# alevar/tiebrush

Hardware: AMD Instinct MI355X
Metric: input alignment records/sec collapsed (tiebrush) + bases/sec covered (tiecov) (higher is better)
Workload: dtype int64; 1 GPU; c3: 64 synthetic sorted BAMs x 5000000 100bp reads per GPU, --clip collapse + tiecov -c -j of the result; records_per_gpu=320000000, groups_out=25086541, parallelism=files-per-rank x1, ranks_seen=1, resident=SoA in HBM before the timed region, contexts=3

## Files before the change

### tiebrush_amd/csrc/collapse.hip

```cpp
#include <stdlib.h>

#include <chrono>

#include "dev_common.hpp"
#include "rx_w64.hpp"
#include "scan_op.hpp"
#include "strategy.hpp"
#include "tbk_internal.h"
#include "wgroup.h"

namespace {

struct EffKey {
  uint32_t khi_h, khi_l;
  int32_t kend;
  uint32_t flag_cnt;
};
struct EffOp {
  __device__ __forceinline__ EffKey operator()(const EffKey& a, const EffKey& b) const {
    uint64_t ak = ((uint64_t)a.khi_h << 32) | a.khi_l, bk = ((uint64_t)b.khi_h << 32) | b.khi_l;
    bool take_b = (b.flag_cnt >> 31) || bk > ak || (bk == ak && b.kend > a.kend);
    EffKey r;
    r.khi_h = take_b ? b.khi_h : a.khi_h;
    r.khi_l = take_b ? b.khi_l : a.khi_l;
// ... 354 lines not shown
  if (i >= n) return;
  const uint32_t sg = rec_sg[i];
  rec_group[i] = sg == 0xFFFFFFFFu ? -1 : (int32_t)ginv[sg];
}


constexpr uint32_t YS_NT = 1024;
constexpr uint32_t YS_NL = 128;
struct YsIn {
  uint32_t ng;
  const uint32_t* gperm;
  const uint32_t* ns;
  const uint32_t* gpoff;
  const uint16_t* pfile;
  const uint64_t* ghi;
  const uint64_t* gfmask;
};
__device__ __forceinline__ uint64_t ys_spread32(uint64_t x) {
  x = (x | (x << 16)) & 0x0000FFFF0000FFFFull;
  x = (x | (x << 8)) & 0x00FF00FF00FF00FFull;
  x = (x | (x << 4)) & 0x0F0F0F0F0F0F0F0Full;
  x = (x | (x << 2)) & 0x3333333333333333ull;
  x = (x | (x << 1)) & 0x5555555555555555ull;
  return x;
}
__device__ __forceinline__ void ys_mask_from_files(uint64_t files, uint32_t c, uint64_t* lo, uint64_t* hi) {
  const uint64_t a = ys_spread32(files & 0xFFFFFFFFull), b = ys_spread32(files >> 32);
  *lo = c == 0u ? a : (c == 1u ? a << 1 : (a | (a << 1)));
  *hi = c == 0u ? b : (c == 1u ? b << 1 : (b | (b << 1)));
}
__device__ __forceinline__ uint64_t wave_bit_transpose(uint64_t x) {
  const uint32_t lane = lane_id();
#define YS_TSTEP(J, M)                                                                     \
  {                                                                                        \
    const uint64_t tt = ((uint64_t)(uint32_t)__shfl_xor((int)(uint32_t)(x >> 32), J, 64) << 32) | (uint32_t)__shfl_xor((int)(uint32_t)x, J, 64); \
    x = (lane & J) ? (((tt >> J) & M) | (x & ~M)) : ((x & M) | ((tt & M) << J));           \
  }
  YS_TSTEP(32, 0x00000000FFFFFFFFull)
  YS_TSTEP(16, 0x0000FFFF0000FFFFull)
  YS_TSTEP(8, 0x00FF00FF00FF00FFull)
  YS_TSTEP(4, 0x0F0F0F0F0F0F0F0Full)
  YS_TSTEP(2, 0x3333333333333333ull)
  YS_TSTEP(1, 0x5555555555555555ull)
#undef YS_TSTEP
  return x;
}
struct YsAgg {
  uint32_t first_tid, last_tid;
  int32_t mx;
  uint32_t whole;
};
__device__ __forceinline__ YsAgg ys_combine(const YsAgg& a, const YsAgg& b) {
  if (b.last_tid == 0u) return a;
  if (a.last_tid == 0u) return b;
  YsAgg r;
  r.first_tid = a.first_tid;
  r.last_tid = b.last_tid;
  const bool joins = b.whole && b.first_tid == a.last_tid;
  r.mx = joins ? (a.mx > b.mx ? a.mx : b.mx) : b.mx;
  r.whole = joins ? a.whole : 0u;
  return r;
}
struct YsCells {
  uint32_t (*a)[YS_NL];
  uint32_t (*b)[YS_NL];
  int32_t (*m)[YS_NL];
  __device__ __forceinline__ YsAgg get(uint32_t x, uint32_t c) const { return YsAgg{a[x][c] & 0x7FFFFFFFu, b[x][c], m[x][c], a[x][c] >> 31}; }
  __device__ __forceinline__ void put(uint32_t x, uint32_t c, const YsAgg& v) const {
    a[x][c] = v.first_tid | (v.whole << 31);
    b[x][c] = v.last_tid;
    m[x][c] = v.mx;
  }
};
__device__ __forceinline__ YsAgg ys_chain_cells(const YsCells& P, uint32_t c, YsAgg run) {
  for (uint32_t x = 0; x < YS_NT / 64; ++x) {
    const YsAgg mine = P.get(x, c);
    P.put(x, c, run);
    run = ys_combine(run, mine);
  }
  return run;
}
__global__ __launch_bounds__(YS_NT) void yd_lcount_k(YsIn S, const uint4* __restrict__ gpk , uint32_t ntiles,
                                                     uint32_t* __restrict__ table , uint4* __restrict__ agg ,
                                                     uint64_t* __restrict__ gfiles ) {
  __shared__ uint64_t wb[YS_NT / 64][YS_NL];
  __shared__ uint32_t g_tid[YS_NT];
  __shared__ int32_t g_e1[YS_NT];
  __shared__ uint32_t pa[YS_NT / 64][YS_NL], pb[YS_NT / 64][YS_NL];
  __shared__ int32_t pm[YS_NT / 64][YS_NL];
  const YsCells P{pa, pb, pm};
  uint64_t lo = 0, hi = 0;
  {
    const uint32_t o = blockIdx.x * YS_NT + threadIdx.x;
    if (o < S.ng) {
      const uint32_t sg = S.gperm[o];
      const uint32_t c = (uint32_t)S.ghi[sg] & 3u;
      const uint32_t n = S.gfmask ? 0u : S.ns[sg], p0 = S.gfmask ? 0u : S.gpoff[sg];
      uint64_t files = 0;
      if (S.gfmask)
        files = S.gfmask[sg];
      else
        for (uint32_t i = 0; i < n; ++i) files |= 1ull << S.pfile[p0 + i];
      gfiles[2 * (size_t)o] = files;
      gfiles[2 * (size_t)o + 1] = c;
      ys_mask_from_files(files, c, &lo, &hi);
      const uint4 g = gpk[o];
      g_tid[threadIdx.x] = g.x;
      g_e1[threadIdx.x] = (int32_t)g.z + 1;
    }
  }
  wb[threadIdx.x >> 6][lane_id()] = wave_bit_transpose(lo);
  wb[threadIdx.x >> 6][64u + lane_id()] = wave_bit_transpose(hi);
  __syncthreads();
  for (uint32_t q = threadIdx.x; q < (YS_NT / 64) * YS_NL; q += YS_NT) {
    const uint32_t x = q / YS_NL, c = q % YS_NL;
    YsAgg A{0u, 0u, INT32_MIN, 1u};
    for (uint64_t m = wb[x][c]; m; m &= m - 1) {
      const uint32_t g = x * 64u + (uint32_t)__builtin_ctzll(m);
      A = ys_combine(A, YsAgg{g_tid[g], g_tid[g], g_e1[g], 1u});
    }
    P.put(x, c, A);
  }
  __syncthreads();
  if (threadIdx.x < YS_NL) {
    const uint32_t c = threadIdx.x;
    uint32_t n = 0;
    for (uint32_t x = 0; x < YS_NT / 64; ++x) n += (uint32_t)__builtin_popcountll(wb[x][c]);
    const YsAgg A = ys_chain_cells(P, c, YsAgg{0u, 0u, INT32_MIN, 1u});
    table[(size_t)c * ntiles + blockIdx.x] = n;
    agg[(size_t)c * ntiles + blockIdx.x] = make_uint4(A.first_tid, A.last_tid, (uint32_t)A.mx, A.whole);
  }
}
__global__ __launch_bounds__(256) void yd_lagg_scan_k(uint4* __restrict__ agg, uint32_t ntiles) {
  __shared__ uint4 part[256];
  uint4* row = agg + (size_t)blockIdx.x * ntiles;
  const uint32_t per = (ntiles + 255u) / 256u, i0 = threadIdx.x * per, i1 = i0 + per < ntiles ? i0 + per : ntiles;
  auto un = [](const uint4& v) { return YsAgg{v.x, v.y, (int32_t)v.z, v.w}; };
  auto pk = [](const YsAgg& a) { return make_uint4(a.first_tid, a.last_tid, (uint32_t)a.mx, a.whole); };
  YsAgg A{0u, 0u, INT32_MIN, 1u};
  for (uint32_t i = i0; i < i1; ++i) A = ys_combine(A, un(row[i]));
  part[threadIdx.x] = pk(A);
  __syncthreads();
  if (threadIdx.x == 0) {
    YsAgg run{0u, 0u, INT32_MIN, 1u};
    for (uint32_t q = 0; q < 256; ++q) {
      const YsAgg mine = un(part[q]);
      part[q] = pk(run);
      run = ys_combine(run, mine);
    }
  }
  __syncthreads();
  YsAgg run = un(part[threadIdx.x]);
  for (uint32_t i = i0; i < i1; ++i) {
    const YsAgg mine = un(row[i]);
    row[i] = pk(run);
    run = ys_combine(run, mine);
  }
}
__global__ __launch_bounds__(1024) void yd_lscan_k(uint32_t* __restrict__ table, uint32_t ntiles, uint64_t* __restrict__ totals,
                                                   unsigned long long* __restrict__ nit ) {
  __shared__ uint32_t sm[16];
  __shared__ uint32_t carry_s;
  uint32_t* row = table + (size_t)blockIdx.x * ntiles;
  constexpr uint32_t E = 8;
  if (threadIdx.x == 0) carry_s = 0;
  __syncthreads();
  for (uint32_t base = 0; base < ntiles; base += 1024 * E) {
    const uint32_t i0 = base + threadIdx.x * E;
    uint32_t v[E], s = 0;
#pragma unroll
    for (uint32_t e = 0; e < E; ++e) {
      v[e] = i0 + e < ntiles ? row[i0 + e] : 0u;
      s += v[e];
    }
    uint32_t tot;
    uint32_t ex = carry_s + block_excl_sum<uint32_t, 1024>(s, sm, &tot);
#pragma unroll
    for (uint32_t e = 0; e < E; ++e) {
      if (i0 + e < ntiles) row[i0 + e] = ex;
      ex += v[e];
    }
    __syncthreads();
    if (threadIdx.x == 0) carry_s += tot;
    __syncthreads();
  }
  if (threadIdx.x == 0) {
    totals[blockIdx.x] = carry_s;
    atomicAdd(nit, (unsigned long long)carry_s);
  }
}

struct YdWords {
  const uint64_t* w64;
  const uint32_t* w32;
  __device__ __forceinline__ uint32_t group(uint32_t t) const { return w32 ? w32[t] : (uint32_t)w64[t]; }
};
struct YdItems {
  uint4* pk;
  uint32_t* nex;
  uint2* se = nullptr;
  const uint32_t* gxoff = nullptr;
  __device__ __forceinline__ uint4 rec(uint32_t t) const {
    if (se) {
      const uint2 a = se[t];
      return make_uint4(0u, a.x, a.y, 0u);
    }
    return pk[t];
  }
  __device__ __forceinline__ uint32_t xo_of(const uint4& it, uint32_t group) const { return se ? gxoff[group] : it.w; }
  __device__ __forceinline__ uint32_t tidp1(uint32_t t) const { return reinterpret_cast<const uint32_t*>(pk)[4 * (size_t)t]; }
  __device__ __forceinline__ int32_t start(uint32_t t) const { return (int32_t) reinterpret_cast<const uint32_t*>(pk)[4 * (size_t)t + 1]; }
// ... 19 lines not shown
  *s1 = 0;
  if ((h32 >> 30) == 2u) {
    const uint32_t op = h32 & 0xFu;
    return (op == C_M || op == C_D || op == 7u || op == 8u || op == 0xFu) ? 1u : 0u;
  }
  if ((h32 >> 30) == 3u) {
    const uint32_t a = (h32 >> 20) & 0x3FFu, g = h32 & 0xFFFFFu;
    *e0 = st + a - 1u;
    *s1 = st + a + g;
    return 2u;
  }
  return 0u;
}

__global__ void yd_groups_k(ColIn I, uint32_t ng, const uint32_t* __restrict__ gperm, GroupAcc G, const uint64_t* __restrict__ shi,
                            const uint64_t* __restrict__ slo, YdGroups Q) {
  uint32_t o = blockIdx.x * blockDim.x + threadIdx.x;
  if (o >= ng) return;
  uint32_t sg = gperm[o];
  uint32_t q = G.first[sg];
  uint64_t h = shi[q], l = slo[q];
  int32_t st = (int32_t)(uint32_t)((h >> 2) & 0x7FFFFFFFull);
  const uint32_t tidp1 = (uint32_t)(h >> 33);
  const uint32_t en = (uint32_t)(st + (int32_t)(uint32_t)(l >> 32) - 1);
  uint32_t e0, s1;
  const uint32_t nk = yd_exons_from_key(l, (uint32_t)st, en, &e0, &s1);
  int nex = (int)nk;
  if (nex == 0) {
    const uint32_t r = (uint32_t)(G.rep[sg] & 0xFFFFFFFFull);
    walk_exons(I.pos[r], I.cig + I.cig_off[r], I.cig_off[r + 1] - I.cig_off[r], [](int, int) {}, &nex);
  }
  uint32_t xw = (uint32_t)nex;
  if (nk == 2u) {
    const uint32_t a = e0 - (uint32_t)st + 1u, g = s1 - e0 - 1u;
    if (a < (1u << 10) && g < (1u << 20)) xw = YD_X2 | (a << 20) | g;
  }
  Q.nex[o] = yd_nex_far(xw) ? (uint32_t)nex : 0u;
  Q.pk[o] = make_uint4(tidp1, (uint32_t)st, en, xw);
}

__global__ void yd_gexons_k(ColIn I, uint32_t ng, const uint32_t* __restrict__ gperm, GroupAcc G, const uint64_t* __restrict__ slo, YdGroups Q,
                            uint32_t* __restrict__ ex_s, uint32_t* __restrict__ ex_e) {
  uint32_t o = blockIdx.x * blockDim.x + threadIdx.x;
  if (o >= ng) return;
  const uint4 pk = Q.pk[o];
  if (!yd_nex_far(pk.w)) return;
  const uint32_t sg = gperm[o];
  uint32_t w = Q.xoff[o];
  {
    uint32_t e0, s1;
    const uint32_t nk = yd_exons_from_key(slo[G.first[sg]], pk.y, pk.z, &e0, &s1);
    if (nk) {
      ex_s[w] = pk.y;
      ex_e[w] = e0;
      if (nk == 2u) {
        ex_s[w + 1] = s1;
        ex_e[w + 1] = pk.z;
      }
      return;
    }
  }
  uint32_t r = (uint32_t)(G.rep[sg] & 0xFFFFFFFFull);
  int nex = 0;
  walk_exons(I.pos[r], I.cig + I.cig_off[r], I.cig_off[r + 1] - I.cig_off[r],
             [&](int es, int ee) {
               ex_s[w] = (uint32_t)es;
               ex_e[w] = (uint32_t)ee;
               ++w;
             },
             &nex);
}

struct YdEmit {
  YdGroups Q;
  YdItems Y;
  __device__ __forceinline__ void operator()(uint32_t t, uint64_t w) const {
    const uint32_t o = (uint32_t)w;
    const uint4 g = Q.pk[o];
    Y.pk[t] = make_uint4(g.x, g.y, g.z, Q.xoff[o]);
    Y.nex[t] = g.w;
  }
};

__device__ __forceinline__ uint32_t ys_select(uint64_t v, uint32_t r) {
  const uint32_t lo = (uint32_t)v, cl = (uint32_t)__builtin_popcount(lo);
  const bool up = r >= cl;
  const uint32_t w = up ? (uint32_t)(v >> 32) : lo;
  r = up ? r - cl : r;
  uint32_t pos = 0;
#pragma unroll
  for (uint32_t st = 16; st >= 1; st >>= 1) {
    const uint32_t c = (uint32_t)__builtin_popcount((w >> pos) & ((1u << st) - 1u));
    const bool go = r >= c;
    r = go ? r - c : r;
    pos = go ? pos + st : pos;
  }
  return pos + (up ? 32u : 0u);
}
__global__ __launch_bounds__(YS_NT) void yd_lscatter_k(YsIn S, uint32_t ntiles, const uint32_t* __restrict__ table, const uint64_t* __restrict__ totals,
                                                       const uint4* __restrict__ agg, const uint64_t* __restrict__ gfiles, YdGroups Q, YdItems Y,
                                                       uint32_t* __restrict__ item) {
  __shared__ uint32_t base[YS_NL];
  __shared__ uint32_t pre[YS_NL + 1];
  __shared__ uint64_t wb[YS_NT / 64][YS_NL];
  __shared__ uint64_t hb[YS_NT / 64][YS_NL];
  __shared__ uint32_t ltot[YS_NL];
  __shared__ uint32_t lsum[YS_NL];
  __shared__ uint4 grec[YS_NT];
  __shared__ uint32_t gnex[YS_NT];
  __shared__ uint32_t pa[YS_NT / 64][YS_NL], pb[YS_NT / 64][YS_NL];
  __shared__ int32_t pm[YS_NT / 64][YS_NL];
  const YsCells P{pa, pb, pm};
  const uint32_t t = threadIdx.x, w = t >> 6;
  if (t < YS_NL) ltot[t] = (uint32_t)totals[t];
  const uint32_t o = blockIdx.x * YS_NT + t;
  uint64_t lo = 0, hi = 0;
  if (o < S.ng) ys_mask_from_files(gfiles[2 * (size_t)o], (uint32_t)gfiles[2 * (size_t)o + 1], &lo, &hi);
  wb[w][lane_id()] = wave_bit_transpose(lo);
  wb[w][64u + lane_id()] = wave_bit_transpose(hi);
  if (o < S.ng) {
    const uint4 g = Q.pk[o];
    grec[t] = make_uint4(g.x, g.y, g.z, Q.xoff[o]);
    gnex[t] = g.w;
  }
  __syncthreads();
  for (uint32_t q = t; q < (YS_NT / 64) * YS_NL; q += YS_NT) {
    const uint32_t x = q / YS_NL, c = q % YS_NL;
    YsAgg A{0u, 0u, INT32_MIN, 1u};
    for (uint64_t m = wb[x][c]; m; m &= m - 1) {
      const uint4 g = grec[x * 64u + (uint32_t)__builtin_ctzll(m)];
      A = ys_combine(A, YsAgg{g.x, g.x, (int32_t)g.z + 1, 1u});
    }
    P.put(x, c, A);
  }
  __syncthreads();
  if (t < YS_NL) {
    uint32_t b = 0;
    for (uint32_t c = 0; c < t; ++c) b += ltot[c];
    base[t] = b + table[(size_t)t * ntiles + blockIdx.x];
    uint32_t n = 0;
    for (uint32_t x = 0; x < YS_NT / 64; ++x) n += (uint32_t)__builtin_popcountll(wb[x][t]);
    lsum[t] = n;
    const uint4 av = agg[(size_t)t * ntiles + blockIdx.x];
    (void)ys_chain_cells(P, t, YsAgg{av.x, av.y, (int32_t)av.z, av.w});
  }
  __syncthreads();
  for (uint32_t q = t; q < (YS_NT / 64) * YS_NL; q += YS_NT) {
    const uint32_t x = q / YS_NL, c = q % YS_NL;
    YsAgg A = P.get(x, c);
    uint64_t heads = 0;
    for (uint64_t m = wb[x][c]; m; m &= m - 1) {
      const uint32_t bit = (uint32_t)__builtin_ctzll(m);
      const uint4 g = grec[x * 64u + bit];
      if (A.last_tid == 0u || g.x != A.last_tid || (int32_t)g.y > A.mx) heads |= 1ull << bit;
      A = ys_combine(A, YsAgg{g.x, g.x, (int32_t)g.z + 1, 1u});
    }
    hb[x][c] = heads;
  }
  __syncthreads();
  if (t < 64) {
    const uint32_t a = lsum[2 * t], b = lsum[2 * t + 1];
    const uint32_t inc = wave_incl_sum(a + b);
    pre[2 * t] = inc - a - b;
    pre[2 * t + 1] = inc - b;
    if (t == 63) pre[YS_NL] = inc;
  } else if (t < 64 + YS_NL) {
    const uint32_t c = t - 64;
    uint32_t run = 0;
    for (uint32_t x = 0; x < YS_NT / 64; ++x) {
      pa[x][c] = run;
      run += (uint32_t)__builtin_popcountll(wb[x][c]);
    }
  }
  __syncthreads();
  const uint32_t T = pre[YS_NL];
  for (uint32_t idx = t; idx < T; idx += YS_NT) {
    uint32_t c = 0;
#pragma unroll
    for (uint32_t st = 64; st >= 1; st >>= 1) c = pre[c + st] <= idx ? c + st : c;
    uint32_t r = idx - pre[c];
    const uint32_t rank = r;
    uint32_t x = 0;
#pragma unroll
    for (uint32_t st = YS_NT / 128; st >= 1; st >>= 1) x = pa[x + st][c] <= r ? x + st : x;
    r -= pa[x][c];
    const uint32_t bit = ys_select(wb[x][c], r);
    const uint32_t g = x * 64u + bit;
    const uint32_t pos = base[c] + rank;
    if (Y.se)
      Y.se[pos] = make_uint2(grec[g].y, grec[g].z);
    else
      Y.pk[pos] = grec[g];
    Y.nex[pos] = gnex[g] | ((uint32_t)((hb[x][c] >> bit) & 1ull) << 31);
    item[pos] = blockIdx.x * YS_NT + g;
  }
}

struct SegMaxY {
  int32_t mx;
  uint32_t flag;
};
struct SegMaxYOp {
  __device__ __forceinline__ SegMaxY operator()(const SegMaxY& a, const SegMaxY& b) const {
    SegMaxY r;
    r.mx = b.flag ? b.mx : (a.mx > b.mx ? a.mx : b.mx);
    r.flag = a.flag | b.flag;
    return r;
  }
};
struct YdLoad {
  const uint64_t* list;
  YdItems Y;
  __device__ __forceinline__ bool list_head(uint32_t t) const {
    return t == 0 || (list[t] >> 32) != (list[t - 1] >> 32) || Y.tidp1(t) != Y.tidp1(t - 1);
  }
  __device__ __forceinline__ SegMaxY operator()(uint32_t t) const {
    SegMaxY s;
    s.mx = Y.end(t) + 1;
    s.flag = list_head(t) ? 1u : 0u;
    return s;
  }
};
struct HeadNex {
  uint32_t h, n;
};
struct HeadNexOp {
  __device__ __forceinline__ HeadNex operator()(const HeadNex& a, const HeadNex& b) const { return HeadNex{a.h + b.h, a.n + b.n}; }
};
struct YdAux {
  YdItems Y;
  __device__ __forceinline__ int2 operator()(uint32_t t) const { return make_int2(Y.start(t), (int)yd_nex_count(Y.nex[t])); }
};
struct YdHead {
  __device__ __forceinline__ HeadNex operator()(uint32_t, const SegMaxY& v, const SegMaxY&, const SegMaxY& ex, const int2& a) const {
    return HeadNex{(v.flag || a.x > ex.mx) ? 1u : 0u, (uint32_t)a.y};
  }
};
struct YdStore {
  YdItems Y;
  uint32_t *chain_first, *chain_noff;
  uint64_t* totals;
  uint32_t nit;
  __device__ __forceinline__ void operator()(uint32_t t, const SegMaxY&, const SegMaxY&, const SegMaxY&, const HeadNex& v, const HeadNex& ex,
                                             const int2&) const {
    if (v.h) {
      chain_first[ex.h] = t;
      chain_noff[ex.h] = ex.n;
    }
    if (t + 1 == nit) {
      totals[0] = ex.h + v.h;
      totals[1] = ex.n + v.n;
    }
  }
};

constexpr uint32_t YN_NT = 256, YN_ROWS = 4, YN_TILE = YN_NT * 4 * YN_ROWS;
__device__ __forceinline__ uint4 yn_load(const uint32_t* __restrict__ w, uint64_t i, uint32_t nit) {
  if (i + 3 < nit) return *reinterpret_cast<const uint4*>(w + i);
  uint4 v = make_uint4(0u, 0u, 0u, 0u);
  if (i < nit) v.x = w[i];
  if (i + 1 < nit) v.y = w[i + 1];
  if (i + 2 < nit) v.z = w[i + 2];
  return v;
}
__global__ __launch_bounds__(YN_NT) void yn_reduce_k(const uint32_t* __restrict__ w, uint32_t nit, unsigned long long* __restrict__ part) {
  __shared__ unsigned long long sm[YN_NT / 64];
  unsigned long long acc = 0;
#pragma unroll
  for (uint32_t r = 0; r < YN_ROWS; ++r) {
    const uint4 v = yn_load(w, (uint64_t)blockIdx.x * YN_TILE + ((uint64_t)r * YN_NT + threadIdx.x) * 4u, nit);
    const uint32_t h = (v.x >> 31) + (v.y >> 31) + (v.z >> 31) + (v.w >> 31);
    const uint32_t n = yd_nex_count(v.x) + yd_nex_count(v.y) + yd_nex_count(v.z) + yd_nex_count(v.w);
    acc += ((unsigned long long)h << 32) + n;
  }
  acc = wave_sum(acc);
  if (lane_id() == 0) sm[threadIdx.x >> 6] = acc;
  __syncthreads();
// ... 793 lines not shown
  uint32_t sg = gperm[o];
  rep[o] = (uint32_t)(G.rep[sg] & 0xFFFFFFFFull);
  if (rep_effend) rep_effend[o] = effend ? effend[rep[o]] : (int32_t)(uint32_t)(G.rep[sg] >> 32);
  yc[o] = G.yc[sg];
  yx[o] = (G.yxin ? (int64_t)G.yxin[sg] : 0ll) + (int64_t)G.ns[sg];
  uint32_t q = G.first[sg];
  int32_t st = (int32_t)(uint32_t)((shi[q] >> 2) & 0x7FFFFFFFull);
  if (g_start) g_start[o] = st;
  if (g_end) g_end[o] = st + (int32_t)(uint32_t)(slo[q] >> 32) - 1;
  if (g_key) {
    const uint64_t lo = slo[q];
    const uint32_t h32 = (uint32_t)lo;
    uint32_t shape = 0;
    if (strategy == TBK_STRAT_CIGAR || strategy == TBK_STRAT_CLIP) {
      if (h32 == (0x80000000u | C_M)) shape = 0x80000000u;
      if ((h32 >> 30) == 3u) shape = h32;
    }
    g_key[2 * (size_t)o] = shi[q];
    g_key[2 * (size_t)o + 1] = (lo & 0xFFFFFFFF00000000ull) | shape;
  }
}
__global__ void col_recgroup_k(const uint64_t* __restrict__ pm, const uint32_t* __restrict__ val, const uint32_t* __restrict__ sgid,
                               const uint32_t* __restrict__ ginv, int32_t* __restrict__ rec_group) {
  const uint32_t m = (uint32_t)*pm;
  uint32_t q = blockIdx.x * blockDim.x + threadIdx.x;
  if (q < m) rec_group[val[q]] = (int32_t)ginv[sgid[q]];
}

__global__ void col_init_groups_k(const uint64_t* __restrict__ png, GroupAcc G, int32_t* __restrict__ g_yd) {
  const uint32_t ng = (uint32_t)*png;
  uint32_t g = blockIdx.x * blockDim.x + threadIdx.x;
  if (g >= ng) return;
  G.yc[g] = 0.0;
  G.ns[g] = 0;
  G.yxin[g] = 0;
  G.ydin[g] = 0;
  G.rep[g] = ~0ull;
  g_yd[g] = 0;
}

struct YdJob {
  ColIn I;
  uint32_t m, ng, cap;
  const uint32_t* val;
  const uint8_t* flags;
  const uint16_t* fidx;
  const uint32_t *sgid, *ginv, *gperm;
  GroupAcc G;
  const uint64_t *shi, *slo;
  int32_t* g_yd;
  int32_t* out_yd;
  bool win = false;
  uint32_t np = 0;
  const uint16_t* pfile = nullptr;
  const uint32_t *pgrp = nullptr, *gpoff = nullptr;
  const uint64_t* gfmask = nullptr;
};

}

int tbk_collapse_yd_run(tbk_ctx* ctx, void* jobp) {
  const YdJob J = *(const YdJob*)jobp;
  delete (YdJob*)jobp;
  const uint32_t B = 256;
  const uint32_t m = J.m, ng = J.ng;
  const ColIn& I = J.I;
  uint64_t* sc = ctx->d_scalars;
  TBK_HIP(hipSetDevice(ctx->device));
  const bool ph = ctx->dbg.phases;
  const auto p0 = std::chrono::steady_clock::now();
  auto p1 = p0, p2 = p0, p3 = p0;
  auto since = [](std::chrono::steady_clock::time_point a) { return std::chrono::duration<double, std::milli>(std::chrono::steady_clock::now() - a).count(); };
  TBK_HIP(hipMemsetAsync(sc, 0, 32 * sizeof(uint64_t), ctx->stream));
  {
    uint32_t *icnt = nullptr, *ioff = nullptr, *ocnt = nullptr, *ooff = nullptr;
    uint64_t nit64;
    const bool by_list = J.win && (!J.pgrp || tbk_yd_by_list(ctx, I.k));
    static_assert(YS_NL == 128, "tbk_yd_by_list (wgroup.h) knows the number of lists");
    const uint32_t ys_tiles = cdiv(ng, YS_NT);
    const YsIn S{ng, J.gperm, J.G.ns, J.gpoff, J.pfile, J.shi, J.gfmask};
    uint32_t* ys_table = nullptr;
    uint4* ys_agg = nullptr;
    uint64_t* ys_totals = nullptr;
    uint64_t* ys_files = nullptr;
    uint32_t *yd_d = nullptr, *ys_item = nullptr;
    YdGroups Q{};
    if (by_list) {
      Q.pk = ws_alloc<uint4>(ctx, ng);
      Q.nex = ws_alloc<uint32_t>(ctx, ng);
      Q.xoff = ws_alloc<uint32_t>(ctx, ng);
      ys_table = ws_alloc<uint32_t>(ctx, (size_t)YS_NL * ys_tiles);
      ys_agg = ws_alloc<uint4>(ctx, (size_t)YS_NL * ys_tiles);
      ys_totals = ws_alloc<uint64_t>(ctx, YS_NL + 1);
      ys_files = ws_alloc<uint64_t>(ctx, 2 * (size_t)ng);
      if (!Q.xoff || !ys_table || !ys_agg || !ys_totals || !ys_files) return TBK_ENOMEM;
      TBK_LAUNCH(ctx, "yd_groups", yd_groups_k, cdiv(ng, B), B, 0, I, ng, J.gperm, J.G, J.shi, J.slo, Q);
      TBK_TRY(tbk_exscan_u32(ctx, Q.nex, Q.xoff, ng, sc + 5));
      TBK_LAUNCH(ctx, "yd_lcount", yd_lcount_k, ys_tiles, YS_NT, 0, S, Q.pk, ys_tiles, ys_table, ys_agg, ys_files);
      TBK_LAUNCH(ctx, "yd_lscan", yd_lscan_k, YS_NL, 1024, 0, ys_table, ys_tiles, ys_totals, (unsigned long long*)(sc + 2));
      TBK_LAUNCH(ctx, "yd_lscan", yd_lagg_scan_k, YS_NL, 256, 0, ys_agg, ys_tiles);
    } else if (J.win) {
      ocnt = ws_alloc<uint32_t>(ctx, ng);
      ooff = ws_alloc<uint32_t>(ctx, ng);
      if (!ooff) return TBK_ENOMEM;
      TBK_LAUNCH(ctx, "yd_gcount", yd_gcount_w_k, cdiv(ng, B), B, 0, ng, J.gperm, J.G, J.shi, ocnt);
      TBK_TRY(tbk_exscan_u32(ctx, ocnt, ooff, ng, sc + 2));
    } else {
      icnt = ws_alloc<uint32_t>(ctx, m);
      ioff = ws_alloc<uint32_t>(ctx, m);
      if (!ioff) return TBK_ENOMEM;
      TBK_LAUNCH(ctx, "yd_count", yd_count_k, cdiv(m, B), B, 0, I, m, J.val, J.flags, J.fidx, icnt);
      TBK_TRY(tbk_exscan_u32(ctx, icnt, ioff, m, sc + 2));
    }
    TBK_HIP(hipMemcpyAsync(ctx->h_scalars, sc, 16 * sizeof(uint64_t), hipMemcpyDeviceToHost, ctx->stream));
    TBK_HIP(hipStreamSynchronize(ctx->stream));
    nit64 = ctx->h_scalars[2];
    p1 = p2 = p3 = std::chrono::steady_clock::now();
    if (nit64 >= (1ull << 32)) return TBK_E2BIG;
    const uint32_t nit = (uint32_t)nit64;
    if (nit) {
      uint64_t* iv = by_list ? nullptr : ws_alloc<uint64_t>(ctx, nit);
      uint64_t* iv2 = by_list ? nullptr : ws_alloc<uint64_t>(ctx, nit);
      uint32_t* io = by_list ? ws_alloc<uint32_t>(ctx, nit) : nullptr;
      yd_d = by_list ? ws_alloc<uint32_t>(ctx, nit) : nullptr;
      if (by_list && (!io || !yd_d)) return TBK_ENOMEM;
      ys_item = io;
      YdItems Y;
      if (by_list) {
        Y.pk = nullptr;
        Y.se = ws_alloc<uint2>(ctx, nit);
        Y.gxoff = Q.xoff;
        if (!Y.se) return TBK_ENOMEM;
      } else {
        Y.pk = ws_alloc<uint4>(ctx, nit);
      }
      Y.nex = ws_alloc<uint32_t>(ctx, nit);
      uint32_t* noff = ws_alloc<uint32_t>(ctx, nit);
      uint32_t* chain_first = ws_alloc<uint32_t>(ctx, nit);
      if (!chain_first) return TBK_ENOMEM;
      if (by_list) {
      } else if (J.win) {
        TBK_LAUNCH(ctx, "yd_fill", yd_fill_w_k, cdiv(J.np, B), B, 0, J.np, J.pfile, J.pgrp, J.gpoff, J.ginv, ooff, J.shi, iv);
      } else {
        ocnt = ws_alloc<uint32_t>(ctx, ng);
        ooff = ws_alloc<uint32_t>(ctx, ng);
        if (!ooff) return TBK_ENOMEM;
        TBK_LAUNCH(ctx, "yd_gcount", yd_gcount_k, cdiv(ng, B), B, 0, ng, m, J.gperm, J.G, ioff, icnt, ocnt);
        TBK_TRY(tbk_exscan_u32(ctx, ocnt, ooff, ng, nullptr));
        TBK_LAUNCH(ctx, "yd_fill", yd_fill_k, cdiv(m, B), B, 0, I, m, J.val, J.flags, J.fidx, J.sgid, J.ginv, ioff, ooff, J.G, iv);
      }
      if (!by_list) {
        Q.pk = ws_alloc<uint4>(ctx, ng);
        Q.nex = ws_alloc<uint32_t>(ctx, ng);
        Q.xoff = ws_alloc<uint32_t>(ctx, ng);
        if (!Q.xoff) return TBK_ENOMEM;
        TBK_LAUNCH(ctx, "yd_groups", yd_groups_k, cdiv(ng, B), B, 0, I, ng, J.gperm, J.G, J.shi, J.slo, Q);
        TBK_TRY(tbk_exscan_u32(ctx, Q.nex, Q.xoff, ng, sc + 5));
      }
      if (by_list) {
        TBK_LAUNCH(ctx, "yd_scatter", yd_lscatter_k, ys_tiles, YS_NT, 0, S, ys_tiles, ys_table, ys_totals, ys_agg, ys_files, Q, Y, io);
      } else {
        uint32_t bits = 1;
        while ((1ull << bits) < 2ull * I.k) ++bits;
        TBK_TRY(tbk_radix_sort_w64_emit(ctx, &iv, &iv2, nit, ((1ull << bits) - 1ull) << 32, true, YdEmit{Q, Y}, "yd_scatter"));
      }
      if (by_list) {
        const uint32_t ynb = cdiv(nit, YN_TILE);
        unsigned long long* ypart = ws_alloc<unsigned long long>(ctx, ynb);
        if (!ypart) return TBK_ENOMEM;
        TBK_LAUNCH(ctx, "yd_number", yn_reduce_k, ynb, YN_NT, 0, Y.nex, nit, ypart);
        TBK_LAUNCH(ctx, "yd_number", yn_spine_k, 1, 1024, 0, ypart, ynb, sc + 3);
        TBK_LAUNCH(ctx, "yd_number", yn_emit_k, ynb, YN_NT, 0, Y.nex, nit, ypart, chain_first, noff);
      } else {
        YdLoad ld{iv, Y};
        YdAux ax{Y};
        YdHead hd{};
        YdStore st{Y, chain_first, noff, sc + 3, nit};
        SegMaxY ident{INT32_MIN, 0u};
        TBK_TRY((scan_two_run<8, SegMaxY, SegMaxYOp, HeadNex, HeadNexOp, YdLoad, YdAux, YdHead, YdStore>(ctx, "yd_chains", nit, ld, ax, hd, st, SegMaxYOp{}, ident,
                                                                                              HeadNexOp{}, HeadNex{0u, 0u})));
      }
      TBK_HIP(hipMemcpyAsync(ctx->h_scalars, sc, 16 * sizeof(uint64_t), hipMemcpyDeviceToHost, ctx->stream));
      TBK_HIP(hipStreamSynchronize(ctx->stream));
      const uint32_t nchains = (uint32_t)ctx->h_scalars[3];
      const uint64_t nnodes = ctx->h_scalars[4], ngex = ctx->h_scalars[5];
      p2 = p3 = std::chrono::steady_clock::now();
      if (nnodes >= (1ull << 31)) return TBK_E2BIG;
      SegNodes N;
      N.s = ws_alloc<uint32_t>(ctx, nnodes + 1);
      N.e = ws_alloc<uint32_t>(ctx, nnodes + 1);
      N.nx = ws_alloc<int32_t>(ctx, nnodes + 1);
      uint32_t* ex_s = ws_alloc<uint32_t>(ctx, ngex + 1);
      uint32_t* ex_e = ws_alloc<uint32_t>(ctx, ngex + 1);
      uint32_t* ids_lane = ws_alloc<uint32_t>(ctx, nchains);
      uint32_t* ids_long = ws_alloc<uint32_t>(ctx, nchains);
      uint32_t* ids_over = ws_alloc<uint32_t>(ctx, nchains);
      uint32_t* bcnt = ws_alloc<uint32_t>(ctx, 4 * YD_NB + 4);
      if (!ids_over || !bcnt) return TBK_ENOMEM;
      uint32_t* bcur = bcnt + 2 * YD_NB;
      uint32_t* n_wave = bcur + 2 * YD_NB;
      uint32_t* n_over = n_wave + 1;
      TBK_HIP(hipMemsetAsync(bcnt, 0, (4 * YD_NB + 4) * sizeof(uint32_t), ctx->stream));
      TBK_LAUNCH(ctx, "yd_gexons", yd_gexons_k, cdiv(ng, B), B, 0, I, ng, J.gperm, J.G, J.slo, Q, ex_s, ex_e);
      const uint32_t wave_min = ctx->dbg.yd_wave_min ? ctx->dbg.yd_wave_min : YD_WAVE_MIN_DEFAULT;
      const uint32_t bgrid = ctx->dbg.yd_bgrid ? ctx->dbg.yd_bgrid : std::min(cdiv(nchains, B), YD_BGRID);
      TBK_LAUNCH(ctx, "yd_classify", yd_bucket_count_k, bgrid, B, 0, nchains, nit, wave_min, chain_first, bcnt);
      TBK_LAUNCH(ctx, "yd_classify", yd_bucket_off_k, 1, 1, 0, bcnt, bcur);
      TBK_LAUNCH(ctx, "yd_classify", yd_bucket_fill_k, bgrid, B, 0, nchains, nit, wave_min, chain_first, bcur, ids_lane, ids_long);
      uint32_t* hc = (uint32_t*)(ctx->h_scalars + 24);
      TBK_HIP(hipMemcpyAsync(hc, n_wave, sizeof(uint32_t), hipMemcpyDeviceToHost, ctx->stream));
      TBK_HIP(hipStreamSynchronize(ctx->stream));
      const uint32_t n_long = hc[0], n_lane = nchains - n_long;
      p3 = std::chrono::steady_clock::now();
      const bool literal = ctx->dbg.yd_literal;
      if (literal) {
        if (n_long) TBK_HIP(hipMemcpyAsync(ids_over, ids_long, (size_t)n_long * 4, hipMemcpyDeviceToDevice, ctx->stream));
        if (n_lane) TBK_HIP(hipMemcpyAsync(ids_over + n_long, ids_lane, (size_t)n_lane * 4, hipMemcpyDeviceToDevice, ctx->stream));
        hc[1] = nchains;
        TBK_HIP(hipMemcpyAsync(n_over, hc + 1, sizeof(uint32_t), hipMemcpyHostToDevice, ctx->stream));
        TBK_HIP(hipStreamSynchronize(ctx->stream));
      }
      hipStream_t aux = n_lane && n_long && !literal ? tbk_aux_stream(ctx) : nullptr;
      if (n_long && !literal) {
        hipStream_t keep = ctx->stream;
        if (aux) ctx->stream = aux;
        TBK_LAUNCH(ctx, "yd_wave", yd_wave_k, n_long, 64, 0, ids_long, n_wave, nchains, nit, chain_first, Y, YdWords{iv, io}, noff, ex_s, ex_e, J.g_yd,
                   yd_d, ids_over, n_over);
        ctx->stream = keep;
        if (aux) TBK_HIP(hipEventRecord(ctx->aux_done, aux));
      }
      if (n_lane && !literal)
        TBK_LAUNCH(ctx, "yd_lane", yd_lane_k<8>, cdiv(n_lane, 64), 64, 0, ids_lane, n_lane, nchains, nit, chain_first, Y, YdWords{iv, io}, ex_s, ex_e, J.g_yd,
                   yd_d, ids_over, n_over);
      if (n_long && aux) TBK_HIP(hipStreamWaitEvent(ctx->stream, ctx->aux_done, 0));
      TBK_LAUNCH(ctx, "yd_run_overflow", yd_run_k, cdiv(nchains, 64), 64, 0, ids_over, n_over, nchains, nit, chain_first, Y, YdWords{iv, io}, noff, ex_s, ex_e,
                 N, J.g_yd, yd_d);
    }
    if (by_list) {
      TBK_LAUNCH(ctx, "yd_gather", yd_lgather_k, ys_tiles, 512, 0, ng, ys_tiles, ys_table, ys_totals, yd_d, ys_item, J.gperm, J.G, J.cap, J.out_yd);
      TBK_HIP(hipStreamSynchronize(ctx->stream));
      if (ph)
        fprintf(stderr, "YD stage ms: counts %.1f | placement + numbering %.1f | buckets %.1f | list machines + gather %.1f (arena %.2f of %.2f GB, %zu overflow chunks)\n",
                std::chrono::duration<double, std::milli>(p1 - p0).count(), std::chrono::duration<double, std::milli>(p2 - p1).count(),
// ... 729 lines not shown
```

Baseline: 20.17 billion records/s.

## Restructure list scatter to walk per-cell bitmasks and stage items in LDS

The count kernel now saves its wave-transposed per-cell bitmasks to global memory, so the scatter kernel reads them directly instead of rebuilding them from per-group file masks. The scatter kernel no longer assigns one output item per thread and locates it with two binary searches plus a bit-select. Instead, each thread walks its two cells in order, computing head flags inline, and writes packed entries into a large LDS staging buffer in chunks. A coalesced pass then writes them out. This removes the per-item search cost and the separate heads pass, but adds a bigger LDS footprint, a serial walk per cell, and extra global traffic for the saved masks. The scatter now always writes Y.se, dropping the old Y.pk fallback.

```diff
diff --git a/tiebrush_amd/csrc/collapse.hip b/tiebrush_amd/csrc/collapse.hip
--- a/tiebrush_amd/csrc/collapse.hip
+++ b/tiebrush_amd/csrc/collapse.hip
@@ -460,7 +460,7 @@
 }
 __global__ __launch_bounds__(YS_NT) void yd_lcount_k(YsIn S, const uint4* __restrict__ gpk , uint32_t ntiles,
                                                      uint32_t* __restrict__ table , uint4* __restrict__ agg ,
-                                                     uint64_t* __restrict__ gfiles ) {
+                                                     uint64_t* __restrict__ gwb ) {
   __shared__ uint64_t wb[YS_NT / 64][YS_NL];
   __shared__ uint32_t g_tid[YS_NT];
   __shared__ int32_t g_e1[YS_NT];
@@ -479,16 +479,21 @@
         files = S.gfmask[sg];
       else
         for (uint32_t i = 0; i < n; ++i) files |= 1ull << S.pfile[p0 + i];
-      gfiles[2 * (size_t)o] = files;
-      gfiles[2 * (size_t)o + 1] = c;
       ys_mask_from_files(files, c, &lo, &hi);
       const uint4 g = gpk[o];
       g_tid[threadIdx.x] = g.x;
       g_e1[threadIdx.x] = (int32_t)g.z + 1;
     }
   }
-  wb[threadIdx.x >> 6][lane_id()] = wave_bit_transpose(lo);
-  wb[threadIdx.x >> 6][64u + lane_id()] = wave_bit_transpose(hi);
+  {
+    const uint32_t x = threadIdx.x >> 6, l = lane_id();
+    const uint64_t a = wave_bit_transpose(lo), b = wave_bit_transpose(hi);
+    wb[x][l] = a;
+    wb[x][64u + l] = b;
+    uint64_t* out = gwb + (size_t)blockIdx.x * (YS_NT / 64) * YS_NL + x * YS_NL;
+    out[l] = a;
+    out[64u + l] = b;
+  }
   __syncthreads();
   for (uint32_t q = threadIdx.x; q < (YS_NT / 64) * YS_NL; q += YS_NT) {
     const uint32_t x = q / YS_NL, c = q % YS_NL;
@@ -503,8 +508,11 @@
   if (threadIdx.x < YS_NL) {
     const uint32_t c = threadIdx.x;
     uint32_t n = 0;
-    for (uint32_t x = 0; x < YS_NT / 64; ++x) n += (uint32_t)__builtin_popcountll(wb[x][c]);
-    const YsAgg A = ys_chain_cells(P, c, YsAgg{0u, 0u, INT32_MIN, 1u});
+    YsAgg A{0u, 0u, INT32_MIN, 1u};
+    for (uint32_t x = 0; x < YS_NT / 64; ++x) {
+      n += (uint32_t)__builtin_popcountll(wb[x][c]);
+      A = ys_combine(A, P.get(x, c));
+    }
     table[(size_t)c * ntiles + blockIdx.x] = n;
     agg[(size_t)c * ntiles + blockIdx.x] = make_uint4(A.first_tid, A.last_tid, (uint32_t)A.mx, A.whole);
   }
@@ -690,117 +698,90 @@
   }
 };
 
-__device__ __forceinline__ uint32_t ys_select(uint64_t v, uint32_t r) {
-  const uint32_t lo = (uint32_t)v, cl = (uint32_t)__builtin_popcount(lo);
-  const bool up = r >= cl;
-  const uint32_t w = up ? (uint32_t)(v >> 32) : lo;
-  r = up ? r - cl : r;
-  uint32_t pos = 0;
-#pragma unroll
-  for (uint32_t st = 16; st >= 1; st >>= 1) {
-    const uint32_t c = (uint32_t)__builtin_popcount((w >> pos) & ((1u << st) - 1u));
-    const bool go = r >= c;
-    r = go ? r - c : r;
-    pos = go ? pos + st : pos;
-  }
-  return pos + (up ? 32u : 0u);
-}
-__global__ __launch_bounds__(YS_NT) void yd_lscatter_k(YsIn S, uint32_t ntiles, const uint32_t* __restrict__ table, const uint64_t* __restrict__ totals,
-                                                       const uint4* __restrict__ agg, const uint64_t* __restrict__ gfiles, YdGroups Q, YdItems Y,
-                                                       uint32_t* __restrict__ item) {
-  __shared__ uint32_t base[YS_NL];
+constexpr uint32_t YS_CAP = 15360;
+constexpr uint32_t YS_NC = (YS_NT / 64) * YS_NL;
+static_assert(YS_NC == 2 * YS_NT && YS_CAP >= 4 * YS_NC, "the staging array holds the cells' aggregates and counts first");
+__global__ __launch_bounds__(YS_NT) void yd_lscatter_k(uint32_t ng, uint32_t ntiles, const uint32_t* __restrict__ table,
+                                                       const uint64_t* __restrict__ totals, const uint4* __restrict__ agg,
+                                                       const uint64_t* __restrict__ gwb , YdGroups Q,
+                                                       YdItems Y, uint32_t* __restrict__ item) {
+  __shared__ uint32_t off[YS_NL];
   __shared__ uint32_t pre[YS_NL + 1];
-  __shared__ uint64_t wb[YS_NT / 64][YS_NL];
-  __shared__ uint64_t hb[YS_NT / 64][YS_NL];
-  __shared__ uint32_t ltot[YS_NL];
   __shared__ uint32_t lsum[YS_NL];
+  __shared__ uint32_t lbase[YS_NL];
   __shared__ uint4 grec[YS_NT];
-  __shared__ uint32_t gnex[YS_NT];
-  __shared__ uint32_t pa[YS_NT / 64][YS_NL], pb[YS_NT / 64][YS_NL];
-  __shared__ int32_t pm[YS_NT / 64][YS_NL];
-  const YsCells P{pa, pb, pm};
-  const uint32_t t = threadIdx.x, w = t >> 6;
-  if (t < YS_NL) ltot[t] = (uint32_t)totals[t];
+  __shared__ uint32_t stage[YS_CAP];
+  const YsCells P{reinterpret_cast<uint32_t(*)[YS_NL]>(stage), reinterpret_cast<uint32_t(*)[YS_NL]>(stage + YS_NC),
+                  reinterpret_cast<int32_t(*)[YS_NL]>(stage + 2 * YS_NC)};
+  uint32_t(*pa)[YS_NL] = reinterpret_cast<uint32_t(*)[YS_NL]>(stage + 3 * YS_NC);
+  const uint32_t t = threadIdx.x, c = t % YS_NL, x0 = t / YS_NL, x1 = x0 + YS_NT / YS_NL;
+  const uint64_t* col = gwb + (size_t)blockIdx.x * YS_NC;
+  const uint64_t m0 = col[t], m1 = col[YS_NT + t];
+  if (t < YS_NL) lbase[t] = (uint32_t)totals[t];
   const uint32_t o = blockIdx.x * YS_NT + t;
-  uint64_t lo = 0, hi = 0;
-  if (o < S.ng) ys_mask_from_files(gfiles[2 * (size_t)o], (uint32_t)gfiles[2 * (size_t)o + 1], &lo, &hi);
-  wb[w][lane_id()] = wave_bit_transpose(lo);
-  wb[w][64u + lane_id()] = wave_bit_transpose(hi);
-  if (o < S.ng) {
-    const uint4 g = Q.pk[o];
-    grec[t] = make_uint4(g.x, g.y, g.z, Q.xoff[o]);
-    gnex[t] = g.w;
-  }
+  if (o < ng) grec[t] = Q.pk[o];
   __syncthreads();
-  for (uint32_t q = t; q < (YS_NT / 64) * YS_NL; q += YS_NT) {
-    const uint32_t x = q / YS_NL, c = q % YS_NL;
+  auto fold = [&](uint64_t m, uint32_t x) {
+    pa[x][c] = (uint32_t)__builtin_popcountll(m);
     YsAgg A{0u, 0u, INT32_MIN, 1u};
-    for (uint64_t m = wb[x][c]; m; m &= m - 1) {
+    for (; m; m &= m - 1) {
       const uint4 g = grec[x * 64u + (uint32_t)__builtin_ctzll(m)];
       A = ys_combine(A, YsAgg{g.x, g.x, (int32_t)g.z + 1, 1u});
     }
     P.put(x, c, A);
-  }
+  };
+  fold(m0, x0);
+  fold(m1, x1);
   __syncthreads();
   if (t < YS_NL) {
-    uint32_t b = 0;
-    for (uint32_t c = 0; c < t; ++c) b += ltot[c];
-    base[t] = b + table[(size_t)t * ntiles + blockIdx.x];
-    uint32_t n = 0;
-    for (uint32_t x = 0; x < YS_NT / 64; ++x) n += (uint32_t)__builtin_popcountll(wb[x][t]);
-    lsum[t] = n;
     const uint4 av = agg[(size_t)t * ntiles + blockIdx.x];
     (void)ys_chain_cells(P, t, YsAgg{av.x, av.y, (int32_t)av.z, av.w});
-  }
-  __syncthreads();
-  for (uint32_t q = t; q < (YS_NT / 64) * YS_NL; q += YS_NT) {
-    const uint32_t x = q / YS_NL, c = q % YS_NL;
-    YsAgg A = P.get(x, c);
-    uint64_t heads = 0;
-    for (uint64_t m = wb[x][c]; m; m &= m - 1) {
-      const uint32_t bit = (uint32_t)__builtin_ctzll(m);
-      const uint4 g = grec[x * 64u + bit];
-      if (A.last_tid == 0u || g.x != A.last_tid || (int32_t)g.y > A.mx) heads |= 1ull << bit;
-      A = ys_combine(A, YsAgg{g.x, g.x, (int32_t)g.z + 1, 1u});
-    }
-    hb[x][c] = heads;
+    uint32_t run = 0;
+    for (uint32_t x = 0; x < YS_NT / 64; ++x) {
+      const uint32_t n = pa[x][t];
+      pa[x][t] = run;
+      run += n;
+    }
+    lsum[t] = run;
   }
   __syncthreads();
   if (t < 64) {
-    const uint32_t a = lsum[2 * t], b = lsum[2 * t + 1];
-    const uint32_t inc = wave_incl_sum(a + b);
+    const uint32_t a = lsum[2 * t], b = lsum[2 * t + 1], inc = wave_incl_sum(a + b);
+    const uint32_t ta = lbase[2 * t], tb = lbase[2 * t + 1], tinc = wave_incl_sum(ta + tb);
     pre[2 * t] = inc - a - b;
     pre[2 * t + 1] = inc - b;
     if (t == 63) pre[YS_NL] = inc;
-  } else if (t < 64 + YS_NL) {
-    const uint32_t c = t - 64;
-    uint32_t run = 0;
-    for (uint32_t x = 0; x < YS_NT / 64; ++x) {
-      pa[x][c] = run;
-      run += (uint32_t)__builtin_popcountll(wb[x][c]);
-    }
+    off[2 * t] = tinc - ta - tb + table[(size_t)(2 * t) * ntiles + blockIdx.x] - (inc - a - b);
+    off[2 * t + 1] = tinc - tb + table[(size_t)(2 * t + 1) * ntiles + blockIdx.x] - (inc - b);
   }
   __syncthreads();
-  const uint32_t T = pre[YS_NL];
-  for (uint32_t idx = t; idx < T; idx += YS_NT) {
-    uint32_t c = 0;
-#pragma unroll
-    for (uint32_t st = 64; st >= 1; st >>= 1) c = pre[c + st] <= idx ? c + st : c;
-    uint32_t r = idx - pre[c];
-    const uint32_t rank = r;
-    uint32_t x = 0;
-#pragma unroll
-    for (uint32_t st = YS_NT / 128; st >= 1; st >>= 1) x = pa[x + st][c] <= r ? x + st : x;
-    r -= pa[x][c];
-    const uint32_t bit = ys_select(wb[x][c], r);
-    const uint32_t g = x * 64u + bit;
-    const uint32_t pos = base[c] + rank;
-    if (Y.se)
-      Y.se[pos] = make_uint2(grec[g].y, grec[g].z);
-    else
-      Y.pk[pos] = grec[g];
-    Y.nex[pos] = gnex[g] | ((uint32_t)((hb[x][c] >> bit) & 1ull) << 31);
-    item[pos] = blockIdx.x * YS_NT + g;
+  const YsAgg A0 = P.get(x0, c), A1 = P.get(x1, c);
+  const uint32_t s0 = pre[c] + pa[x0][c], s1 = pre[c] + pa[x1][c], T = pre[YS_NL];
+  for (uint32_t r0 = 0; r0 < T; r0 += YS_CAP) {
+    __syncthreads();
+    const uint32_t r1 = r0 + YS_CAP;
+    auto walk = [&](uint64_t m, uint32_t x, YsAgg A, uint32_t i) {
+      if (i >= r1 || i + (uint32_t)__builtin_popcountll(m) <= r0) return;
+      for (; m && i < r1; m &= m - 1, ++i) {
+        const uint32_t g = x * 64u + (uint32_t)__builtin_ctzll(m);
+        const uint4 v = grec[g];
+        const bool head = A.last_tid == 0u || v.x != A.last_tid || (int32_t)v.y > A.mx;
+        A = ys_combine(A, YsAgg{v.x, v.x, (int32_t)v.z + 1, 1u});
+        if (i >= r0) stage[i - r0] = g | (c << 10) | ((uint32_t)head << 17);
+      }
+    };
+    walk(m0, x0, A0, s0);
+    walk(m1, x1, A1, s1);
+    __syncthreads();
+    const uint32_t n = T - r0 < YS_CAP ? T - r0 : YS_CAP;
+    for (uint32_t i = t; i < n; i += YS_NT) {
+      const uint32_t e = stage[i], g = e & (YS_NT - 1u), l = (e >> 10) & (YS_NL - 1u);
+      const uint4 v = grec[g];
+      const uint32_t pos = off[l] + r0 + i;
+      Y.se[pos] = make_uint2(v.y, v.z);
+      Y.nex[pos] = v.w | ((e >> 17) << 31);
+      item[pos] = blockIdx.x * YS_NT + g;
+    }
   }
 }
 
@@ -1760,7 +1741,7 @@
     uint32_t* ys_table = nullptr;
     uint4* ys_agg = nullptr;
     uint64_t* ys_totals = nullptr;
-    uint64_t* ys_files = nullptr;
+    uint64_t* ys_wb = nullptr;
     uint32_t *yd_d = nullptr, *ys_item = nullptr;
     YdGroups Q{};
     if (by_list) {
@@ -1770,11 +1751,11 @@
       ys_table = ws_alloc<uint32_t>(ctx, (size_t)YS_NL * ys_tiles);
       ys_agg = ws_alloc<uint4>(ctx, (size_t)YS_NL * ys_tiles);
       ys_totals = ws_alloc<uint64_t>(ctx, YS_NL + 1);
-      ys_files = ws_alloc<uint64_t>(ctx, 2 * (size_t)ng);
-      if (!Q.xoff || !ys_table || !ys_agg || !ys_totals || !ys_files) return TBK_ENOMEM;
+      ys_wb = ws_alloc<uint64_t>(ctx, (size_t)ys_tiles * YS_NC);
+      if (!Q.xoff || !ys_table || !ys_agg || !ys_totals || !ys_wb) return TBK_ENOMEM;
       TBK_LAUNCH(ctx, "yd_groups", yd_groups_k, cdiv(ng, B), B, 0, I, ng, J.gperm, J.G, J.shi, J.slo, Q);
       TBK_TRY(tbk_exscan_u32(ctx, Q.nex, Q.xoff, ng, sc + 5));
-      TBK_LAUNCH(ctx, "yd_lcount", yd_lcount_k, ys_tiles, YS_NT, 0, S, Q.pk, ys_tiles, ys_table, ys_agg, ys_files);
+      TBK_LAUNCH(ctx, "yd_lcount", yd_lcount_k, ys_tiles, YS_NT, 0, S, Q.pk, ys_tiles, ys_table, ys_agg, ys_wb);
       TBK_LAUNCH(ctx, "yd_lscan", yd_lscan_k, YS_NL, 1024, 0, ys_table, ys_tiles, ys_totals, (unsigned long long*)(sc + 2));
       TBK_LAUNCH(ctx, "yd_lscan", yd_lagg_scan_k, YS_NL, 256, 0, ys_agg, ys_tiles);
     } else if (J.win) {
@@ -1836,7 +1817,7 @@
         TBK_TRY(tbk_exscan_u32(ctx, Q.nex, Q.xoff, ng, sc + 5));
       }
       if (by_list) {
-        TBK_LAUNCH(ctx, "yd_scatter", yd_lscatter_k, ys_tiles, YS_NT, 0, S, ys_tiles, ys_table, ys_totals, ys_agg, ys_files, Q, Y, io);
+        TBK_LAUNCH(ctx, "yd_scatter", yd_lscatter_k, ys_tiles, YS_NT, 0, ng, ys_tiles, ys_table, ys_totals, ys_agg, ys_wb, Q, Y, io);
       } else {
         uint32_t bits = 1;
         while ((1ull << bits) < 2ull * I.k) ++bits;
```

Result: faster. 20.63 billion records/s, median of 6 (+2.3%).
